# Farofeiro231/LiDAR_SLAM

Hardware: AMD Instinct MI355X
Metric: scans/sec (RANSAC+UKF, 720-pt scans) at 1/2/4/8 MI355X + HBM GB/s vs peak (higher is better)
Workload: dtype f64; 1 GPU; C3: 4096 synthetic 720-pt scans per GPU, chunked 7x100+20; RANSAC (100 trials, 20 mm, mt19937 hypotheses) + landmark association + UKF predict/update (n=3, L=20); scans_per_gpu=4096, trials=100, landmarks=20, hyp=mt19937, parallelism=dp1 (scan shards, no collective)

## Files before the change

lidar_slam_amd/csrc/lidarslam.hip:

```cpp
#include <hip/hip_runtime.h>
#include <math.h>
#include "lslam_host_math.h"
#include <stdio.h>
#include <stdlib.h>
#include <string.h>
#include <algorithm>
#include <atomic>
#include <mutex>
#include <new>
#include <string>
#include <vector>

#include "../../include/lidarslam.h"
#include "lslam_express.h"
#include "lslam_rng.h"
#include "lslam_rng_pipe.h"
#include "lslam_ransac.h"
#include "lslam_ukf.h"
#include "lslam_wave.h"

using namespace lslam;

static_assert(sizeof(lslam_chunk_model) == 112, "chunk model ABI");

__device__ __attribute__((noinline)) double2 polar_xy(double th, double d) {
    const double ang = -th * (LS_PI / 180.0) + LS_PI / 2.0;
    return make_double2(d * cos(ang), d * sin(ang));
}

struct PtSrc {
    const double2 *xy;
    const double *th, *dd;
    __device__ __forceinline__ double2 operator[](int64_t i) const { return xy ? xy[i] : polar_xy(th[i], dd[i]); }
    __device__ __forceinline__ PtSrc operator+(int64_t o) const {
        PtSrc r = *this;
        if (xy) r.xy += o;
        else { r.th += o; r.dd += o; }
        return r;
    }
};
__device__ __forceinline__ PtSrc batch_points(const lslam_scan_batch &B) {
    return PtSrc{(const double2 *)B.xy, B.theta_deg, B.dist_mm};
}
__device__ __forceinline__ void stage_points(const lslam_scan_batch &B, int p0, int N, double2 *P, int lane) {
    if (B.xy) {
        const double2 *src = (const double2 *)B.xy + p0;
        for (int p = lane; p < N; p += 64) P[p] = src[p];
    } else {
        for (int p = lane; p < N; p += 64) P[p] = polar_xy(B.theta_deg[p0 + p], B.dist_mm[p0 + p]);
    }
}
static_assert(sizeof(lslam_landmark) == 56, "landmark ABI");

__device__ __forceinline__ int owning_scan(const lslam_scan_batch &B, int c) {
    const int g = (int)(((int64_t)c * B.n_scans) / (B.n_chunks > 0 ? B.n_chunks : 1));
    if (g < B.n_scans && B.scan_chunk_off[g] <= c && c < B.scan_chunk_off[g + 1]) return uni(g);
    int lo = 0, hi = B.n_scans;
    while (hi - lo > 1) {
        const int mid = (lo + hi) >> 1;
        if (B.scan_chunk_off[mid] <= c) lo = mid;
        else hi = mid;
    }
    return uni(lo);
}

enum { MODE_RANSAC = 1, MODE_ASSOC = 2, MODE_UKF = 4, MODE_HYP_ONLY = 8, MODE_POST = 16 };

typedef float cut_t;
struct ChunkCut {
    double tq;
    double margin;
    cut_t c_lo, c_hi;
    int finite;
    int scan;
};

struct KArgs {
    lslam_scan_batch b;
    double ecut;
    double ecut_q;
    double thr;
    double tol_a, tol_b, tol_dist;
    double tol_dist_sq;
    uint64_t philox_seed;
    int T;
    int hyp_source;
    int life;
    int off_pts, off_key, off_ring, off_draws, off_cnt, off_tied, off_tsum;
    int off_vstack, off_nstack, off_snap, off_lmk, off_vis, off_mask, off_corg, off_zobs;
    int corg_cap;
    int off_recs;
    int off_ukf;
    int off_j1;
    int pts_cap;
    int lmk_cap;
    int hist_cap;
    UkfConst ukf;
    void *jbuf;
    int j8;
    int res_g;
    int32_t *draws_scr;
    uint32_t *state_scr;
    int off_blk, off_nxt, off_vtmp, off_stage;
    int rng_pipe_bytes;
    int off_stbl;
    const uint32_t *rt_all;
    const uint32_t *seed_state;
    int ep_d0, ep_nd;
    int ep_count;
    size_t slot_jbytes;
    int fixup;
    const uint8_t *spec_dirty_in;
    uint8_t *spec_dirty_out;
    int write_yproj;
    int lmk_reg;
    int32_t *cnt_scr;
    double *models;
    int cnt_blocks;
    const ChunkCut *cuts;
    unsigned long long *dbg;
    unsigned long long *wcen;
    unsigned int *wcen_n;
    unsigned int wcen_cap;
    unsigned int call_seq;
};

enum { WC_RNG_PARSER = 1, WC_RNG_HELPER, WC_RESOLVE, WC_CHUNK, WC_FIXUP, WC_POST, WC_UKF };
#if defined(LSLAM_STAMPS) || defined(LSLAM_CENSUS)
struct WaveCensus {
    const KArgs &a;
    uint32_t kid;
    uint64_t t0;
    __device__ WaveCensus(const KArgs &a_, uint32_t kid_) : a(a_), kid(kid_), t0(__builtin_amdgcn_s_memrealtime()) {}
    __device__ ~WaveCensus() {
        if (!a.wcen || (threadIdx.x & 63) != 0) return;
        const uint64_t t1 = __builtin_amdgcn_s_memrealtime();
// ... 132 lines not shown
        const int p = pb + lane;
        const double2 q = P[p < N ? p : 0];
        const bool h = p < N && resid2(q, mw) < ecut;
        const uint64_t bm = ballot(h);
        if (p < N) mk[p] = h ? 1 : 0;
        if (h) P[nin + (int)mbcnt(bm)] = q;
        nin += popc64(bm);
    }
    __syncthreads();
    o.n_inl = nin;
    o.last_inl = nin - 1;
    if (nin == 0) {
        o.flags |= LSLAM_NO_INLIERS;
        return o;
    }
    if (nin == 1) {
        o.flags |= LSLAM_EST_FAIL;
        return o;
    }
    const Model f = (nin == 2) ? model2(P[0], P[1]) : refit_line(P, nin, lane);
    o.m = f;
    o.flags |= LSLAM_VALID;
    if (f.ux == 0.0) o.flags |= LSLAM_VERTICAL;
    return o;
}

__device__ __forceinline__ double tie_bound(double S, int N, double E2) {
    return ((double)N * E2 + (double)(N + 32) * S) * 0x1p-42;
}

__device__ __forceinline__ double tie_bound_r(double S, int N, double E2, double R) {
    return ((double)N * (E2 + R * (sqrt(E2) + 1.0)) + (double)(N + 32) * S) * 0x1p-42;
}
__device__ __forceinline__ double tie_bound_q(double S, int N, double tq) {
    return ((double)N * tq + (double)(N + 32) * S) * 0x1p-42;
}

typedef unsigned u32x16 __attribute__((ext_vector_type(16)));
typedef unsigned u32x4 __attribute__((ext_vector_type(4)));

template <int OFF = 0>
__device__ __forceinline__ u32x16 sload_4pts(const double2 *p) {
    u32x16 v;
    asm volatile("s_load_dwordx16 %0, %1, %2" : "=s"(v) : "s"(p), "i"(OFF) : "memory");
    return v;
}
__device__ __forceinline__ u32x4 sload_pt(const double2 *p) {
    u32x4 v;
    asm volatile("s_load_dwordx4 %0, %1, 0x0" : "=s"(v) : "s"(p) : "memory");
    return v;
}
__device__ __forceinline__ void swait(u32x16 &v) { asm volatile("s_waitcnt lgkmcnt(0)" : "+s"(v)::"memory"); }
__device__ __forceinline__ void swait(u32x4 &v) { asm volatile("s_waitcnt lgkmcnt(0)" : "+s"(v)::"memory"); }
__device__ __forceinline__ double sd(unsigned lo, unsigned hi) {
    return __longlong_as_double((long long)(((unsigned long long)hi << 32) | lo));
}

__device__ __forceinline__ cut_t count_cut(double c) { return __uint_as_float((uint32_t)(__double_as_longlong(c) >> 32)); }
__device__ __forceinline__ bool sure_in(double r, cut_t c) { return __builtin_fabsf(count_cut(r)) < c; }
__device__ __forceinline__ bool maybe_in(double r, cut_t c) { return __builtin_fabsf(count_cut(r)) <= c; }
__device__ __forceinline__ void count_one(double x, double y, double ux, double uy, double k, cut_t c_lo,
                                          cut_t c_hi, int &lo, int &hi, double &S) {
    double t, r;
    asm("v_fma_f64 %0, %1, %2, %3" : "=v"(t) : "s"(y), "v"(ux), "v"(k));
    asm("v_fma_f64 %0, %1, %2, -%3" : "=v"(r) : "s"(x), "v"(uy), "v"(t));
    S = __builtin_fma(r, r, S);
    lo += sure_in(r, c_lo) ? 1 : 0;
    hi += maybe_in(r, c_hi) ? 1 : 0;
    asm volatile("" : "+v"(lo), "+v"(hi));
}

__device__ __forceinline__ void count_four(const u32x16 &A, double ux, double uy, double k, cut_t c_lo, cut_t c_hi,
                                           int &lo, int &hi, double &S) {
    asm volatile(
        "v_fma_f64 v[40:41], %[y0], %[ux], %[k]\n\t"
        "v_fma_f64 v[42:43], %[y1], %[ux], %[k]\n\t"
        "v_fma_f64 v[44:45], %[y2], %[ux], %[k]\n\t"
        "v_fma_f64 v[46:47], %[y3], %[ux], %[k]\n\t"
        "v_fma_f64 v[40:41], %[x0], %[uy], -v[40:41]\n\t"
        "v_fma_f64 v[42:43], %[x1], %[uy], -v[42:43]\n\t"
        "v_fma_f64 v[44:45], %[x2], %[uy], -v[44:45]\n\t"
        "v_fma_f64 v[46:47], %[x3], %[uy], -v[46:47]\n\t"
        "v_cmp_lt_f32_e64 s[80:81], |v41|, %[cl]\n\t"
        "v_cmp_le_f32_e64 s[82:83], |v41|, %[ch]\n\t"
        "v_cmp_lt_f32_e64 s[84:85], |v43|, %[cl]\n\t"
        "v_cmp_le_f32_e64 s[86:87], |v43|, %[ch]\n\t"
        "v_fma_f64 %[S], v[40:41], v[40:41], %[S]\n\t"
        "v_addc_co_u32_e64 %[lo], s[80:81], %[lo], 0, s[80:81]\n\t"
        "v_addc_co_u32_e64 %[hi], s[82:83], %[hi], 0, s[82:83]\n\t"
        "v_fma_f64 %[S], v[42:43], v[42:43], %[S]\n\t"
        "v_cmp_lt_f32_e64 s[80:81], |v45|, %[cl]\n\t"
        "v_cmp_le_f32_e64 s[82:83], |v45|, %[ch]\n\t"
        "v_addc_co_u32_e64 %[lo], s[84:85], %[lo], 0, s[84:85]\n\t"
        "v_addc_co_u32_e64 %[hi], s[86:87], %[hi], 0, s[86:87]\n\t"
        "v_fma_f64 %[S], v[44:45], v[44:45], %[S]\n\t"
        "v_cmp_lt_f32_e64 s[84:85], |v47|, %[cl]\n\t"
        "v_cmp_le_f32_e64 s[86:87], |v47|, %[ch]\n\t"
        "v_addc_co_u32_e64 %[lo], s[80:81], %[lo], 0, s[80:81]\n\t"
        "v_addc_co_u32_e64 %[hi], s[82:83], %[hi], 0, s[82:83]\n\t"
        "v_fma_f64 %[S], v[46:47], v[46:47], %[S]\n\t"
        "v_addc_co_u32_e64 %[lo], s[84:85], %[lo], 0, s[84:85]\n\t"
        "v_addc_co_u32_e64 %[hi], s[86:87], %[hi], 0, s[86:87]"
        : [lo] "+v"(lo), [hi] "+v"(hi), [S] "+v"(S)
        : [x0] "s"(sd(A[0], A[1])), [y0] "s"(sd(A[2], A[3])), [x1] "s"(sd(A[4], A[5])), [y1] "s"(sd(A[6], A[7])),
          [x2] "s"(sd(A[8], A[9])), [y2] "s"(sd(A[10], A[11])), [x3] "s"(sd(A[12], A[13])),
          [y3] "s"(sd(A[14], A[15])), [ux] "v"(ux), [uy] "v"(uy), [k] "v"(k), [cl] "v"(c_lo), [ch] "v"(c_hi)
        : "v40", "v41", "v42", "v43", "v44", "v45", "v46", "v47", "s80", "s81", "s82", "s83", "s84", "s85", "s86",
          "s87");
}

__device__ __forceinline__ void count_points_sgpr(const double2 *gP, int N, double ux, double uy, double k,
                                                  cut_t r_lo, cut_t r_hi, int &lo, int &hi, double &S) {
    const double2 *q = gP;
    if (N >= 8) {
        const double2 *const qlast = gP + ((N >> 3) - 1) * 8;
        u32x16 A = sload_4pts(q), B;
        swait(A);
        while (q != qlast) {
            B = sload_4pts<64>(q);
            count_four(A, ux, uy, k, r_lo, r_hi, lo, hi, S);
            swait(B);
            A = sload_4pts<128>(q);
            count_four(B, ux, uy, k, r_lo, r_hi, lo, hi, S);
            q += 8;
            swait(A);
        }
        B = sload_4pts<64>(q);
        count_four(A, ux, uy, k, r_lo, r_hi, lo, hi, S);
        swait(B);
        count_four(B, ux, uy, k, r_lo, r_hi, lo, hi, S);
        q += 8;
    }
    if (N & 4) {
        u32x16 A = sload_4pts(q);
        swait(A);
        count_four(A, ux, uy, k, r_lo, r_hi, lo, hi, S);
        q += 4;
    }
    for (int r = N & 3; r > 0; r--, q++) {
        u32x4 v = sload_pt(q);
        swait(v);
        count_one(sd(v[0], v[1]), sd(v[2], v[3]), ux, uy, k, r_lo, r_hi, lo, hi, S);
    }
}

__device__ __forceinline__ void count_points_lds(const double2 *P, int N, double ux, double uy, double k, cut_t r_lo,
                                                 cut_t r_hi, int &lo, int &hi, double &S) {
    int p = 0;
    for (; p + 2 <= N; p += 2) {
        const double2 q0 = P[p], q1 = P[p + 1];
        count_one(q0.x, q0.y, ux, uy, k, r_lo, r_hi, lo, hi, S);
        count_one(q1.x, q1.y, ux, uy, k, r_lo, r_hi, lo, hi, S);
    }
    if (p < N) count_one(P[p].x, P[p].y, ux, uy, k, r_lo, r_hi, lo, hi, S);
}

#ifdef LSLAM_STAMPS
#define CH_STAMP(k)                                                            \
    do {                                                                       \
        const uint64_t _t = lslam_stamp();                                     \
        if (chdbg && lane == 0) chdbg[(k)] += _t - _ch_prev;                   \
        _ch_prev = _t;                                                         \
    } while (0)
#define CH_STAMP_DECL uint64_t _ch_prev = lslam_stamp();
#define CH_STAMP_DECL_RESET _ch_prev = lslam_stamp();
#elif defined(LSLAM_CHUNK_EXIT)
#define CH_STAMP_DECL_RESET
#define CH_STAMP(k)                                           \
    do {                                                      \
        if ((k) == LSLAM_CHUNK_EXIT) asm volatile("s_endpgm"); \
    } while (0)
#define CH_STAMP_DECL
#else
#define CH_STAMP_DECL_RESET
#define CH_STAMP(k) do {} while (0)
#define CH_STAMP_DECL
#endif

__device__ __forceinline__ int hkey(double d) {
    const int h = (int)(__double_as_longlong(d) >> 32);
    return h ^ ((h >> 31) & 0x7fffffff);
}
__device__ __forceinline__ double key_up(int k) {
    const int h = k ^ ((k >> 31) & 0x7fffffff);
    return __longlong_as_double((long long)(((unsigned long long)(uint32_t)h << 32) | (h >= 0 ? 0xffffffffull : 0ull)));
}
__device__ __forceinline__ bool key_finite(int k) {
    const int h = k ^ ((k >> 31) & 0x7fffffff);
    return (h & 0x7ff00000) != 0x7ff00000;
}
struct BoxAcc {
    int xh = INT_MIN, xl = INT_MAX, yh = INT_MIN, yl = INT_MAX;
    __device__ __forceinline__ void add(double2 q) {
        const int kx = hkey(q.x), ky = hkey(q.y);
        xh = max(xh, kx);
        xl = min(xl, kx);
        yh = max(yh, ky);
        yl = min(yl, ky);
    }
};
__device__ __forceinline__ ChunkCut cut_finish(BoxAcc b, double ecut, double ecut_q);
template <typename PP>
__device__ __forceinline__ ChunkCut chunk_cut(PP P, int N, double ecut, double ecut_q, int lane) {
    BoxAcc b;
    for (int p = lane; p < N; p += 64) b.add(P[p]);
    return cut_finish(b, ecut, ecut_q);
}

template <int CTRL, int ROWS>
// ... 13 lines not shown
__device__ __forceinline__ float hi_units(double s, int d) {
    return __uint_as_float((uint32_t)(__double_as_longlong(s) >> 32) + (uint32_t)d);
}
__device__ __forceinline__ cut_t cut_lo_of(double e) {
    if (!(e > 0.0)) return -1.0f;
    if (e >= 0x1p-100 && e <= 0x1p100) return hi_units((double)__builtin_amdgcn_sqrtf((float)e), -2);
    return count_cut(sq_floor_lt(e));
}
__device__ __forceinline__ cut_t cut_hi_of(double e) {
    if (e >= 0x1p-100 && e <= 0x1p100) return hi_units((double)__builtin_amdgcn_sqrtf((float)e), 2);
    return count_cut(sq_ceil_gt(e));
}

__device__ __forceinline__ ChunkCut cut_from_keys(int kxh, int kxl, int kyh, int kyl, double ecut, double ecut_q) {
    ChunkCut cc;
    cc.finite = key_finite(kxh) && key_finite(kxl) && key_finite(kyh) && key_finite(kyl);
    const double hx = key_up(kxh), lx = key_up(kxl), hy = key_up(kyh), ly = key_up(kyl);
    const double bx = hx + lx, by = hy + ly;
    const double E2 = (bx * bx + by * by) * (1.0 + 0x1p-20);
    const double Rb = (fmax(hx, lx) + fmax(hy, ly)) * (1.0 + 0x1p-40);
    cc.finite = cc.finite && E2 < __builtin_inf();
    cc.scan = 0;
    cc.tq = 0.0;
    cc.margin = 0.0;
    cc.c_lo = count_cut(-1.0);
    cc.c_hi = count_cut(0.0);
    if (cc.finite && ecut < __builtin_inf()) {
        cc.margin = (E2 + ecut + Rb * ecut_q) * 0x1p-42;
        cc.c_lo = cut_lo_of(ecut - cc.margin);
        cc.c_hi = cut_hi_of(ecut + cc.margin);
        const double sE = (double)__builtin_amdgcn_sqrtf((float)E2) * (1.0 + 0x1p-20);
        cc.tq = E2 + Rb * (sE + 1.0);
    }
    return cc;
}
__device__ __forceinline__ ChunkCut cut_finish(BoxAcc b, double ecut, double ecut_q) {
    return cut_from_keys(wave_max_dpp(b.xh), wave_max_dpp(~b.xl), wave_max_dpp(b.yh), wave_max_dpp(~b.yl), ecut,
                         ecut_q);
}

__device__ ChunkOut chunk_consensus(const KArgs &a, double2 *P, const double2 *gP, int N, const int32_t *draws,
                                    int32_t *cnt, int32_t *tied, double *tsum, uint8_t *mk, double *vtmp,
                                    double *vstack, int *nstack, int32_t *cnt_out, int lane, const ChunkCut *pcut,
                                    unsigned long long *chdbg = nullptr) {
    CH_STAMP_DECL
    const int T = a.T;
    const double ecut = a.ecut;
    const ChunkCut cc = pcut ? *pcut : chunk_cut(P, N, ecut, a.ecut_q, lane);
    if (N > 128 || !cc.finite || !(ecut < __builtin_inf()))
        return chunk_ransac(a, P, N, draws, cnt, tied, tsum, mk, vstack, nstack, cnt_out, lane);

    ChunkOut o;
    o.flags = 0;
    o.best = -1;
    o.stop = -1;
    o.n_inl = 0;
    o.last_inl = -1;
    o.n_draws = T + 1;
    const double margin = cc.margin;
    const cut_t c_lo = cc.c_lo, c_hi = cc.c_hi;
    int M = 0;
    CH_STAMP(1);
    for (int tb = 0; tb < T; tb += 64) {
        const int t = tb + lane;
        const int tt = t < T ? t : 0;
        const Model m = model2(P[draws[2 * tt]], P[draws[2 * tt + 1]]);
        const double un = m.ux * m.ux + m.uy * m.uy;
        const bool exact_all = !(fabs(un - 1.0) <= 0x1p-46);
        const double k = __builtin_fma(m.ox, m.uy, -(m.oy * m.ux));
        int lo = 0, hi = 0;
        double S = 0.0;
        if (gP) count_points_sgpr(gP, N, m.ux, m.uy, k, c_lo, c_hi, lo, hi, S);
        else count_points_lds(P, N, m.ux, m.uy, k, c_lo, c_hi, lo, hi, S);
        int c = lo;
        if (exact_all || lo != hi) {
            c = 0;
            for (int q = 0; q < N; q++) {
                const double r = __builtin_fma(P[q].x, m.uy, -__builtin_fma(P[q].y, m.ux, k));
                const double v = r * r;
                bool in = v < ecut;
                if (exact_all || fabs(v - ecut) <= margin) in = resid2(P[q], m) < ecut;
                c += (int)in;
            }
        }
        if (t < T) {
            cnt[t] = c;
            tsum[t] = exact_all ? -1.0 : S;
            if (cnt_out) cnt_out[t] = c;
        }
        M = max(M, wave_max_dpp(t < T ? c : 0));
    }
    M = uni(M);
    CH_STAMP(2);
    __syncthreads();
    int ntied = 0;
    for (int tb = 0; tb < T; tb += 64) {
        const int t = tb + lane;
        const bool h = t < T && cnt[t] == M;
        const uint64_t bm = ballot(h);
        if (h) tied[ntied + (int)mbcnt(bm)] = t;
        ntied += popc64(bm);
    }
    __syncthreads();
    int best = -1;
    if (T > 0) {
        const bool need_sums = ntied > 1 || M == N || !(ecut > 0.0);
        if (!need_sums) {
            best = tied[0];
        } else {
            double U = __builtin_inf();
            for (int k = lane; k < ntied; k += 64) {
                const double S = tsum[tied[k]];
                if (S >= 0.0) U = fmin(U, S + tie_bound_q(S, N, cc.tq));
            }
            U = wave_min_d(U);
            int ncand = 0, cand1 = -1;
            for (int kb = 0; kb < ntied; kb += 64) {
                const int k = kb + lane;
                bool cand = false;
                if (k < ntied) {
                    const double S = tsum[tied[k]];
                    cand = S < 0.0 || S - tie_bound_q(S, N, cc.tq) <= U;
                }
                const uint64_t cm = ballot(cand);
                if (cm && cand1 < 0) cand1 = kb + ffs64(cm);
                ncand += popc64(cm);
            }
            const bool lone = ncand == 1 && M < N && ecut > 0.0;
            if (lone) best = uni(tied[cand1]);
            int bcnt = 0;
            double bsum = __builtin_inf();
            for (int kb = 0; !lone && kb < ntied && o.stop < 0; kb += 64) {
                const int k = kb + lane;
                bool cand = false;
                if (k < ntied) {
                    const double S = tsum[tied[k]];
                    cand = S < 0.0 || S - tie_bound_q(S, N, cc.tq) <= U;
                }
                uint64_t cm = ballot(cand);
                while (cm) {
                    const int bit = ffs64(cm);
                    cm &= cm - 1ull;
                    const int t = uni(tied[kb + bit]);
                    const Model m = model2(P[draws[2 * t]], P[draws[2 * t + 1]]);
                    const double s = pw_sum_regs(P, N, m, lane);
                    if (M > bcnt || (M == bcnt && s < bsum)) {
                        best = t;
                        bcnt = M;
                        bsum = s;
                        if (bsum <= 0.0) {
                            o.stop = t;
                            break;
                        }
                    }
                }
            }
        }
    }
    CH_STAMP(3);
    const ChunkOut of = chunk_finish_fit(a, P, N, draws, mk, uni(best), o, lane);
    CH_STAMP(4);
    return of;
}

__device__ bool finish_chunk(const KArgs &a, const ChunkOut &o, const double2 *P, uint8_t *mk, int p0, int N,
                             lslam_chunk_model &rec, int lane) {
    const lslam_scan_batch &B = a.b;
    const bool valid = (o.flags & LSLAM_VALID) != 0;
    if (!valid)
        for (int p = lane; p < N; p += 64) mk[p] = 0;
    __syncthreads();
    if (B.inlier_mask)
        for (int p = lane; p < N; p += 64) B.inlier_mask[p0 + p] = mk[p];
    rec.n_inliers = valid ? o.n_inl : 0;
    rec.best_trial = o.best;
    rec.n_draws = o.n_draws;
    rec.flags = o.flags;
    if (valid) {
// ... 888 lines not shown
    constexpr int wpg = 4;
    const int nwaves = (k.b.n_scans + per - 1) / per;
    const dim3 grid((unsigned)((nwaves + wpg - 1) / wpg)), block(64 * wpg);
    const int var = (trace ? UKF_VAR_TRACE : 0) | (k.b.ukf_sigmas ? UKF_VAR_SIGMAS : 0);
    switch (fuse ? 0 : var) {
        case 0: hipLaunchKernelGGL(ukf_group_kernel<0>, grid, block, 0, stream, k, Pg, fuse ? 1 : 0, nullptr); break;
        case 1: hipLaunchKernelGGL(ukf_group_kernel<1>, grid, block, 0, stream, k, Pg, 0, trace); break;
        case 2: hipLaunchKernelGGL(ukf_group_kernel<2>, grid, block, 0, stream, k, Pg, 0, nullptr); break;
        default: hipLaunchKernelGGL(ukf_group_kernel<3>, grid, block, 0, stream, k, Pg, 0, trace); break;
    }
}

__global__ __launch_bounds__(64) void seed_kernel(const uint32_t *__restrict__ seeds, int S, uint32_t *__restrict__ out) {
    __builtin_amdgcn_s_setprio(2);
    const int s = (int)blockIdx.x * 64 + (int)threadIdx.x;
    if (s >= S) return;
    uint32_t x = seeds ? seeds[s] : 0u;
    uint32_t *row = out + (size_t)s * MT_N;
#pragma unroll 8
    for (int i = 0; i < MT_N; i++) {
        row[i] = x;
        x = 1812433253u * (x ^ (x >> 30)) + (uint32_t)(i + 1);
    }
}

__global__ __launch_bounds__(64) void cut_lane_kernel(const KArgs a, ChunkCut *__restrict__ out) {
    __builtin_amdgcn_s_setprio(2);
    const lslam_scan_batch &B = a.b;
    const int c = (int)blockIdx.x * 64 + (int)threadIdx.x;
    if (c >= B.n_chunks) return;
    const int p0 = B.chunk_pt_off[c];
    const int N = B.chunk_pt_off[c + 1] - p0;
    BoxAcc b;
    if (B.xy) {
        const double2 *src = (const double2 *)B.xy + p0;
#pragma unroll 4
        for (int p = 0; p < N; p++) b.add(src[p]);
    } else {
        for (int p = 0; p < N; p++) b.add(polar_xy(B.theta_deg[p0 + p], B.dist_mm[p0 + p]));
    }
    ChunkCut cc = cut_from_keys(b.xh, ~b.xl, b.yh, ~b.yl, a.ecut, a.ecut_q);
    int g = (int)(((int64_t)c * B.n_scans) / (B.n_chunks > 0 ? B.n_chunks : 1));
    if (!(g < B.n_scans && B.scan_chunk_off[g] <= c && c < B.scan_chunk_off[g + 1])) {
        int lo = 0, hi = B.n_scans;
        while (hi - lo > 1) {
            const int mid = (lo + hi) >> 1;
            if (B.scan_chunk_off[mid] <= c) lo = mid;
            else hi = mid;
        }
        g = lo;
    }
    cc.scan = g;
    out[c] = cc;
}

constexpr int RNG_PPW = 4;
template <typename JT>
__global__ __launch_bounds__(64 * RNG_PPW) void rng_kernel(const KArgs a) {
    extern __shared__ __attribute__((aligned(16))) unsigned char smem[];
    const int lane = (int)threadIdx.x & 63;
    const int wave = uni((int)threadIdx.x >> 6);
    const lslam_scan_batch &B = a.b;
    const uint32_t D = a.ep_nd > 0 ? (uint32_t)a.ep_nd : (uint32_t)a.T + 1u;
    WAVE_CENSUS(a, WC_RNG_PARSER);
    RngPipe rp;
    {
        unsigned char *base = smem + (size_t)wave * a.rng_pipe_bytes;
        rp.blk = (uint32_t *)(base + a.off_blk);
        rp.have = 0;
        rp.tbl = nullptr;
        rp.tblK = 0;
    }
    int *kslot = (int *)(smem + a.off_stbl);
    uint32_t *stbl = (uint32_t *)(smem + a.off_stbl + 16);
// ... 454 lines not shown
            }
        };
        uint32_t rawA[RW], rawB[RW];
        if (2u <= K) load_group(2u, rawA);
        for (uint32_t ib = 2; ib <= K; ib += 128u * RW) {
            const uint32_t ib2 = ib + 64u * RW;
            if (ib2 <= K) load_group(ib2, rawB);
            walk_group(ib, rawA);
            if (ib2 > K) break;
            if (ib2 + 64u * RW <= K) load_group(ib2 + 64u * RW, rawA);
            walk_group(ib2, rawB);
        }
        if (lane == 0) {
            const uint32_t j1 = (uint32_t)Jd[K - 1u] & 1u;
            int32_t *draws = a.draws_scr + (size_t)c * 2 * Dall + 2 * (size_t)a.ep_d0;
            draws[2 * d] = (int32_t)((j1 == 0u) ? c1 : c0);
            draws[2 * d + 1] = (int32_t)((j1 == 0u) ? c0 : c1);
        }
    }
}

template <int HYP>
__device__ __forceinline__ void chunk_body(const KArgs &a, const int c, unsigned char *smem) {
    const int lane = (int)threadIdx.x;
    const lslam_scan_batch &B = a.b;
    double2 *P = (double2 *)(smem + a.off_pts);
    int32_t *draws = (int32_t *)(smem + a.off_draws);
    int32_t *cnt = (int32_t *)(smem + a.off_cnt);
    int32_t *tied = (int32_t *)(smem + a.off_tied);
    double *tsum = (double *)(smem + a.off_tsum);
    uint8_t *mk = (uint8_t *)(smem + a.off_mask);
    double *vstack = (double *)(smem + a.off_vstack);
    int *nstack = (int *)(smem + a.off_nstack);
    double *vtmp = (double *)(smem + a.off_vtmp);

    const int s = a.cuts ? uni(a.cuts[c].scan) : owning_scan(B, c);
    const int p0 = B.chunk_pt_off[c];
    const int N = B.chunk_pt_off[c + 1] - p0;
    const int T = a.T;
#ifdef LSLAM_STAMPS
    unsigned long long *chdbg = a.dbg ? a.dbg + (size_t)c * 16 : nullptr;
#else
    unsigned long long *chdbg = nullptr;
#endif
    CH_STAMP_DECL
    lslam_chunk_model rec;
    memset(&rec, 0, sizeof(rec));
    rec.best_trial = -1;
    rec.match_index = -1;
    rec.landmark_id = (B.id_base ? B.id_base[s] : 0) + (c - B.scan_chunk_off[s]);
    rec.n_points = N;
    if (N < 3) {
        rec.flags = LSLAM_N_TOO_SMALL;
        if (lane == 0 && B.models) B.models[c] = rec;
        for (int p = lane; p < N; p += 64) {
            if (B.inlier_mask) B.inlier_mask[p0 + p] = 0;
            if (B.y_proj && a.write_yproj) B.y_proj[p0 + p] = 0.0;
        }
        if (B.trial_cnt_out)
            for (int t = lane; t < a.T; t += 64) B.trial_cnt_out[(size_t)c * a.T + t] = 0;
        return;
    }
    const int D = T + 1;
    const int32_t *dr = draws;
    if (HYP == LSLAM_HYP_PHILOX) {
        philox_draws((uint32_t)N, (uint32_t)D, (uint32_t)c, a.philox_seed, draws, lane);
        if (B.draws_out)
            for (int i = lane; i < 2 * D; i += 64) B.draws_out[(size_t)c * 2 * D + i] = draws[i];
    } else {
        const int32_t *h = (HYP == LSLAM_HYP_EXPLICIT ? B.hyp : a.draws_scr) + (size_t)c * 2 * D;
        dr = h;
        if (N <= 128 && B.xy) {
            double2 pv[2];
            const double2 *src = (const double2 *)B.xy + p0;
#pragma unroll
            for (int k = 0; k < 2; k++) pv[k] = (lane + 64 * k < N) ? src[lane + 64 * k] : make_double2(0.0, 0.0);
#pragma unroll
            for (int k = 0; k < 2; k++)
                if (lane + 64 * k < N) P[lane + 64 * k] = pv[k];
        } else {
            stage_points(B, p0, N, P, lane);
        }
        if (HYP == LSLAM_HYP_EXPLICIT && B.draws_out)
            for (int i = lane; i < 2 * D; i += 64) B.draws_out[(size_t)c * 2 * D + i] = h[i];
    }
    CH_STAMP(0);
    if (HYP == LSLAM_HYP_PHILOX) stage_points(B, p0, N, P, lane);
    __syncthreads();
    CH_STAMP(6);
    const double2 *gP = B.xy ? (const double2 *)B.xy + p0 : nullptr;
    const ChunkOut o = chunk_consensus(a, P, gP, N, dr, cnt, tied, tsum, mk, vtmp, vstack, nstack,
                                       B.trial_cnt_out ? B.trial_cnt_out + (size_t)c * T : nullptr, lane,
                                       a.cuts ? a.cuts + c : nullptr, chdbg);
    CH_STAMP_DECL_RESET
    const bool have_model = finish_chunk(a, o, P, mk, p0, N, rec, lane);
    if (B.y_proj && a.write_yproj) chunk_yproj(B.y_proj + p0, P, mk, N, have_model, rec.proj_a, rec.proj_b, lane);
    if (lane == 0 && B.models) B.models[c] = rec;
    CH_STAMP(5);
}

template <int HYP>
__global__ __launch_bounds__(64, 4) void chunk_kernel(const KArgs a) {
    extern __shared__ __attribute__((aligned(16))) unsigned char smem[];
    WAVE_CENSUS(a, WC_CHUNK);
    for (int c = blockIdx.x; c < a.b.n_chunks; c += gridDim.x) {
        chunk_body<HYP>(a, c, smem);
        __syncthreads();
    }
}

constexpr int CNT_TPB = 256;
constexpr int CNT_HYP_BLOCK = 1024;

typedef const __attribute__((address_space(4))) double cdouble_t;

struct ChunkBox {
    double E2;
    bool finite;
};

template <typename Src>
__device__ __forceinline__ void box_partial(const Src src, int N, int tid, int nthr, double2 *P, double &xmn,
                                            double &xmx, double &ymn, double &ymx, bool &fin) {
    xmn = __builtin_inf(); xmx = -__builtin_inf(); ymn = __builtin_inf(); ymx = -__builtin_inf();
// ... 397 lines not shown
```

lidar_slam_amd/csrc/lslam_launch.h:

```cpp
#pragma once
#include <type_traits>

static inline int align16(int x) { return (x + 15) & ~15; }

template <typename F>
static void with_hyp_source(int hyp_source, F &&f) {
    switch (hyp_source) {
        case LSLAM_HYP_PHILOX: f(std::integral_constant<int, LSLAM_HYP_PHILOX>{}); break;
        case LSLAM_HYP_EXPLICIT: f(std::integral_constant<int, LSLAM_HYP_EXPLICIT>{}); break;
        default: f(std::integral_constant<int, LSLAM_HYP_MT19937>{}); break;
    }
}

static int validate_batch(const lslam_scan_batch *b, bool need_points) {
    if (!b) return set_err(LSLAM_ERR_ARG, "batch is NULL");
    if (b->n_scans < 0 || b->n_chunks < 0 || b->n_points < 0) return set_err(LSLAM_ERR_ARG, "negative sizes");
    if (b->n_scans == 0) return LSLAM_OK;
    if (!b->scan_chunk_off || !b->chunk_pt_off) return set_err(LSLAM_ERR_ARG, "missing CSR offsets");
    if (need_points && !b->xy && (!b->theta_deg || !b->dist_mm) && b->n_points > 0)
        return set_err(LSLAM_ERR_ARG, "missing points (xy, or theta_deg + dist_mm)");
    if (b->max_chunk_points < 0 || b->max_scan_chunks < 0) return set_err(LSLAM_ERR_ARG, "bad maxima");
    return LSLAM_OK;
}

// ... 26 lines not shown
#if defined(LSLAM_STAMPS) || defined(LSLAM_CENSUS)
    k.wcen = g_wcen;
    k.wcen_n = g_wcen_n;
    k.wcen_cap = g_wcen_cap;
    k.call_seq = g_call_seq;
#endif
    k.b = *b;
    if (p) {
        if (p->min_samples != 2) return set_err(LSLAM_ERR_UNSUPPORTED, "only min_samples == 2 (ransac_functions.py:11)");
        if (p->residual_threshold < 0) return set_err(LSLAM_ERR_ARG, "`residual_threshold` must be greater than zero");
        if (p->max_trials < 0) return set_err(LSLAM_ERR_ARG, "`max_trials` must be greater than zero");
        if (p->max_trials > 65533) return set_err(LSLAM_ERR_UNSUPPORTED, "max_trials > 65533");
        if (p->hyp_source < 0 || p->hyp_source > 2) return set_err(LSLAM_ERR_ARG, "bad hyp_source");
        if (p->hyp_source == LSLAM_HYP_EXPLICIT && !b->hyp) return set_err(LSLAM_ERR_ARG, "explicit hyp without hyp");
        k.thr = p->residual_threshold;
        k.ecut = lslam_inlier_cutoff(p->residual_threshold);
        k.ecut_q = std::sqrt(k.ecut) * 1.01 + 1.0;
        k.tol_a = p->tol_a;
        k.tol_b = p->tol_b;
        k.tol_dist = p->tol_dist;
        k.tol_dist_sq = sqrt_le_bound(p->tol_dist);
        k.philox_seed = p->philox_seed;
        k.T = p->max_trials;
        k.hyp_source = p->hyp_source;
        k.life = p->life;
    }
    if ((mode & MODE_ASSOC) && b->landmarks && !b->lmk_count) return set_err(LSLAM_ERR_ARG, "landmarks without lmk_count");
    const int N = b->max_chunk_points > 0 ? b->max_chunk_points : 1;
    const int T = k.T;
    int off = 0;
    if (mode & (MODE_RANSAC | MODE_HYP_ONLY)) {
        k.off_pts = off; off += align16(16 * N);
        k.off_key = off; off += align16(4 * 624);
        const int nxt_bytes = 4 * mt_nslot(N) * N;
        const int uni_bytes = max(nxt_bytes, 8 * (T > 0 ? T : 1));
        k.off_ring = off;
        k.off_tsum = off;
        off += align16(uni_bytes);
        k.off_j1 = off;
        off += align16(4 * mt_nslot(N));
        k.off_draws = off; off += align16(8 * (T + 1));
        k.off_cnt = off; off += align16(4 * (T > 0 ? T : 1));
        k.off_tied = off; off += align16(4 * (T > 0 ? T : 1));
        k.off_mask = off; off += align16(N);
        k.off_vstack = off; off += (N > 128) ? align16(8 * 64 * 24) : 0;
        k.off_nstack = off; off += (N > 128) ? align16(4 * 72) : 0;
        k.off_recs = -1;
    } else {
        k.off_mask = off; off += align16(N);
        const int msc = b->max_scan_chunks > 0 ? b->max_scan_chunks : 1;
        if (msc <= 256) {
            k.off_recs = off;
            off += align16((int)sizeof(lslam_chunk_model) * msc) + align16(4 * (msc + 1));
        } else {
            k.off_recs = -1;
        }
    }
    if (u && u->n_landmarks > 0) {
        k.off_ukf = 0;
        off = max(off, align16(8 * UkfLds::doubles(u->n_landmarks)));
    }
    k.hist_cap = b->max_scan_chunks > 0 ? b->max_scan_chunks : 1;
    k.off_snap = off; off += (mode & MODE_RANSAC) ? align16(4 * MT_N) : 0;
    k.corg_cap = k.hist_cap;
    k.off_corg = off; off += align16(16 * k.corg_cap);
    k.off_zobs = off; off += (u && (u->flags & LSLAM_UKF_MAP)) ? align16(16 * k.corg_cap) : 0;
    k.lmk_cap = (mode & MODE_ASSOC) ? b->lmk_capacity : 0;
    if ((mode & MODE_ASSOC) && k.lmk_cap <= 0) return set_err(LSLAM_ERR_ARG, "lmk_capacity must be > 0");
    k.lmk_reg = (mode == MODE_ASSOC && k.lmk_cap > 0 && k.lmk_cap <= 64 && k.off_recs >= 0 &&
                 !(u && (u->flags & LSLAM_UKF_MAP)) && b->landmarks) ? 1 : 0;
    k.off_lmk = off; off += k.lmk_reg ? 0 : align16((int)sizeof(lslam_landmark) * (k.lmk_cap > 0 ? k.lmk_cap : 1));
    k.off_vis = off; off += k.lmk_reg ? 0 : align16(8 * ((k.lmk_cap + 63) / 64 + 1));
    k.pts_cap = N;
// ... 41 lines not shown
        const int mx = 160 * 1024;
        (void)hipFuncSetAttribute((const void *)scan_kernel<0, MODE>, hipFuncAttributeMaxDynamicSharedMemorySize, mx);
        (void)hipFuncSetAttribute((const void *)scan_kernel<1, MODE>, hipFuncAttributeMaxDynamicSharedMemorySize, mx);
        (void)hipFuncSetAttribute((const void *)scan_kernel<2, MODE>, hipFuncAttributeMaxDynamicSharedMemorySize, mx);
        set_max_lds(scan_kernel_w4<LSLAM_HYP_EXPLICIT, MODE>);
    });
    int st = timer_begin(c, timer);
    if (st) return st;
    if (MODE == MODE_UKF && !(k.ukf.flags & LSLAM_UKF_MAP)) {
        launch_ukf_group(k, k.ukf.L, c->stream, false);
        HIPCHK(hipGetLastError());
    } else if (MODE == MODE_ASSOC || MODE == MODE_UKF) {
        hipLaunchKernelGGL((scan_kernel_w4<LSLAM_HYP_EXPLICIT, MODE>), dim3((unsigned)k.b.n_scans), dim3(64), lds,
                           c->stream, k);
        HIPCHK(hipGetLastError());
    } else {
        HIPCHK(launch_mode<MODE>(k, lds, c->stream));
    }
    st = timer_end(c, timer);
    if (st) return st;
    return LSLAM_OK;
}


static int layout_chunk(KArgs &k, const lslam_scan_batch *b, int &lds) {
    const int N = b->max_chunk_points > 0 ? b->max_chunk_points : 1;
    const int T = k.T;
    int off = 0;
    k.off_pts = off; off += align16(16 * N);
    k.off_draws = off; off += (k.hyp_source == LSLAM_HYP_PHILOX) ? align16(8 * (T + 1)) : 0;
    k.off_cnt = off; off += align16(4 * (T > 0 ? T : 1));
    k.off_tied = off; off += align16(4 * (T > 0 ? T : 1));
    k.off_tsum = off; off += align16(8 * (T > 0 ? T : 1));
    k.off_mask = off; off += align16(N);
    k.off_vstack = off; off += (N > 128) ? align16(8 * 64 * 24) : 0;
    k.off_nstack = off; off += (N > 128) ? align16(4 * 72) : 0;
    k.off_vtmp = off;
    lds = off;
    if (lds > 160 * 1024) return set_err(LSLAM_ERR_CAPACITY, "chunk/trial sizes exceed the 160 KiB LDS");
    return LSLAM_OK;
}

static int layout_rng(KArgs &k, const lslam_scan_batch *b, int &lds) {
    const int N = b->max_chunk_points > 3 ? b->max_chunk_points : 3;
    if (N > 65536) return set_err(LSLAM_ERR_UNSUPPORTED, "chunks of more than 65536 points");
    int off = 0;
    k.off_blk = off; off += align16(4 * (2 * 624 + 64));
    k.rng_pipe_bytes = off;
    lds = off * RNG_PPW;
    k.off_stbl = lds;
    lds += 16 + 2 * 4 * RT_DWORDS;
    return LSLAM_OK;
}

static inline unsigned launch_cap(int64_t n) { return (unsigned)(n < (1 << 30) ? (n > 0 ? n : 1) : (1 << 30)); }

template <typename F>
static void set_max_lds(F *fn) {
    hipFuncAttributes at;
    size_t stat = 0;
    if (hipFuncGetAttributes(&at, (const void *)fn) == hipSuccess) stat = at.sharedSizeBytes;
    (void)hipFuncSetAttribute((const void *)fn, hipFuncAttributeMaxDynamicSharedMemorySize, (int)(160 * 1024 - stat));
    (void)hipGetLastError();
}

static int prepare_steps(lslam_ctx *c, KArgs &k, int slot) {
// ... 656 lines not shown
```

lidar_slam_amd/csrc/lslam_rng.h:

```cpp
#pragma once
#include "lslam_wave.h"

namespace lslam {

__device__ __forceinline__ void wave_lds_sync() {
    __builtin_amdgcn_wave_barrier();
    asm volatile("" ::: "memory");
}

constexpr int MT_N = 624;
constexpr int MT_M = 397;
constexpr uint32_t MT_UP = 0x80000000u;
constexpr uint32_t MT_LO = 0x7fffffffu;
constexpr uint32_t MT_MA = 0x9908b0dfu;

__device__ __forceinline__ uint32_t mt_temper(uint32_t y) {
    y ^= (y >> 11);
    y ^= (y << 7) & 0x9d2c5680u;
    y ^= (y << 15) & 0xefc60000u;
    y ^= (y >> 18);
    return y;
}

__device__ __forceinline__ uint32_t mt_mix(uint32_t cur, uint32_t nxt, uint32_t far) {
// ... 75 lines not shown
};

constexpr uint32_t MT_NONE = 0xffffffffu;

#ifdef LSLAM_STAMPS
__device__ __forceinline__ uint64_t lslam_stamp() {
    uint64_t t;
    __builtin_amdgcn_sched_barrier(0);
    asm volatile("s_memtime %0\n\ts_waitcnt lgkmcnt(0)" : "=s"(t)::"memory");
    __builtin_amdgcn_sched_barrier(0);
    return t;
}
#define LSLAM_STAMP_DECL uint64_t _st_prev = lslam_stamp();
#define LSLAM_STAMP(k)                         \
    do {                                       \
        const uint64_t _t = lslam_stamp();     \
        mt.acc[k] += _t - _st_prev;            \
        _st_prev = _t;                         \
    } while (0)
#else
#define LSLAM_STAMP_DECL
#define LSLAM_STAMP(k) \
    do {               \
    } while (0)
#endif

__host__ __device__ inline int mt_resolve_batch(int N) { return N <= 512 ? 4 : 1; }
__host__ __device__ inline int mt_nslot(int N) {
    const int K = N > 2 ? N - 1 : 2;
    int need = mt_resolve_batch(N) + (64 + K - 1) / K;
    int s = 1;
    while (s < need) s <<= 1;
    return s;
}

__device__ __forceinline__ uint32_t nxt_tag(uint32_t d) { return (0xfffeu - d) << 16; }

__device__ __forceinline__ void mt_resolve(const MTWave &mt, uint32_t N, uint32_t smask, uint32_t d0, uint32_t nb,
                                           int32_t *draws, int lane) {
    const uint32_t k = (uint32_t)lane >> 1;
    const uint32_t q = (uint32_t)lane & 1u;
    uint32_t p = q;
    const uint32_t d = d0 + k;
    const uint32_t slot = d & smask;
    const uint32_t tag = nxt_tag(d);
    if (k < nb) {
        const uint32_t *nx = mt.nxt + slot * N;
        for (;;) {
            const uint32_t t = nx[p];
            if ((t & 0xffff0000u) != tag) break;
            p = t & 0xffffu;
        }
    }
    const uint32_t other = (uint32_t)__shfl_xor((int)p, 1);
    if (k < nb && q == 0) {
        const uint32_t j1 = mt.j1s[slot];
        const uint32_t a0 = (j1 == 0u) ? other : p;
        const uint32_t a1 = (j1 == 0u) ? p : other;
        draws[2 * d] = (int32_t)a0;
        draws[2 * d + 1] = (int32_t)a1;
    }
    wave_lds_sync();
}

template <bool FAST>
__device__ void mt_draws_impl(MTWave &mt, uint32_t N, uint32_t D, int32_t *draws, bool store, int lane) {
// ... 147 lines not shown
```

Measured before the change: 6.261 million scans/s.

## Replace per-point residual sum accumulation with closed-form moment-based tie bracket

The inner RANSAC counting loop no longer accumulates the squared residual sum per point. Instead, per-chunk second moments are precomputed in the cut pass, and the sum of squared residuals for each hypothesis line is computed in closed form, together with a rigorous per-trial error bound stored as a float in LDS. This removes an FMA per point per trial from the hot counting loop. In exchange it adds moment accumulation in the prepass, a new LDS buffer and bound logic for tie-breaking. It also risks a fallback to the exact path more often when the bounds are loose, and a wave reduction when no precomputed cuts exist.

```diff
diff --git a/lidar_slam_amd/csrc/lidarslam.hip b/lidar_slam_amd/csrc/lidarslam.hip
--- a/lidar_slam_amd/csrc/lidarslam.hip
+++ b/lidar_slam_amd/csrc/lidarslam.hip
@@ -16,6 +16,7 @@
 #include "lslam_rng.h"
 #include "lslam_rng_pipe.h"
 #include "lslam_ransac.h"
+#include "lslam_tie_moments.h"
 #include "lslam_ukf.h"
 #include "lslam_wave.h"
 
@@ -73,7 +74,10 @@
     cut_t c_lo, c_hi;
     int finite;
     int scan;
+    TieMoments mom;
+    double tm_ok;
 };
+static_assert(sizeof(ChunkCut) == 96 && sizeof(ChunkCut) % 16 == 0, "ChunkCut: six 16-byte rows");
 
 struct KArgs {
     lslam_scan_batch b;
@@ -102,6 +106,7 @@
     int32_t *draws_scr;
     uint32_t *state_scr;
     int off_blk, off_nxt, off_vtmp, off_stage;
+    int off_tbnd;
     int rng_pipe_bytes;
     int off_stbl;
     const uint32_t *rt_all;
@@ -300,9 +305,6 @@
 __device__ __forceinline__ double tie_bound_r(double S, int N, double E2, double R) {
     return ((double)N * (E2 + R * (sqrt(E2) + 1.0)) + (double)(N + 32) * S) * 0x1p-42;
 }
-__device__ __forceinline__ double tie_bound_q(double S, int N, double tq) {
-    return ((double)N * tq + (double)(N + 32) * S) * 0x1p-42;
-}
 
 typedef unsigned u32x16 __attribute__((ext_vector_type(16)));
 typedef unsigned u32x4 __attribute__((ext_vector_type(4)));
@@ -328,18 +330,17 @@
 __device__ __forceinline__ bool sure_in(double r, cut_t c) { return __builtin_fabsf(count_cut(r)) < c; }
 __device__ __forceinline__ bool maybe_in(double r, cut_t c) { return __builtin_fabsf(count_cut(r)) <= c; }
 __device__ __forceinline__ void count_one(double x, double y, double ux, double uy, double k, cut_t c_lo,
-                                          cut_t c_hi, int &lo, int &hi, double &S) {
+                                          cut_t c_hi, int &lo, int &hi) {
     double t, r;
     asm("v_fma_f64 %0, %1, %2, %3" : "=v"(t) : "s"(y), "v"(ux), "v"(k));
     asm("v_fma_f64 %0, %1, %2, -%3" : "=v"(r) : "s"(x), "v"(uy), "v"(t));
-    S = __builtin_fma(r, r, S);
     lo += sure_in(r, c_lo) ? 1 : 0;
     hi += maybe_in(r, c_hi) ? 1 : 0;
     asm volatile("" : "+v"(lo), "+v"(hi));
 }
 
 __device__ __forceinline__ void count_four(const u32x16 &A, double ux, double uy, double k, cut_t c_lo, cut_t c_hi,
-                                           int &lo, int &hi, double &S) {
+                                           int &lo, int &hi) {
     asm volatile(
         "v_fma_f64 v[40:41], %[y0], %[ux], %[k]\n\t"
         "v_fma_f64 v[42:43], %[y1], %[ux], %[k]\n\t"
@@ -353,32 +354,28 @@
         "v_cmp_le_f32_e64 s[82:83], |v41|, %[ch]\n\t"
         "v_cmp_lt_f32_e64 s[84:85], |v43|, %[cl]\n\t"
         "v_cmp_le_f32_e64 s[86:87], |v43|, %[ch]\n\t"
-        "v_fma_f64 %[S], v[40:41], v[40:41], %[S]\n\t"
+        "v_cmp_lt_f32_e64 s[88:89], |v45|, %[cl]\n\t"
+        "v_cmp_le_f32_e64 s[90:91], |v45|, %[ch]\n\t"
         "v_addc_co_u32_e64 %[lo], s[80:81], %[lo], 0, s[80:81]\n\t"
         "v_addc_co_u32_e64 %[hi], s[82:83], %[hi], 0, s[82:83]\n\t"
-        "v_fma_f64 %[S], v[42:43], v[42:43], %[S]\n\t"
-        "v_cmp_lt_f32_e64 s[80:81], |v45|, %[cl]\n\t"
-        "v_cmp_le_f32_e64 s[82:83], |v45|, %[ch]\n\t"
+        "v_cmp_lt_f32_e64 s[80:81], |v47|, %[cl]\n\t"
+        "v_cmp_le_f32_e64 s[82:83], |v47|, %[ch]\n\t"
         "v_addc_co_u32_e64 %[lo], s[84:85], %[lo], 0, s[84:85]\n\t"
         "v_addc_co_u32_e64 %[hi], s[86:87], %[hi], 0, s[86:87]\n\t"
-        "v_fma_f64 %[S], v[44:45], v[44:45], %[S]\n\t"
-        "v_cmp_lt_f32_e64 s[84:85], |v47|, %[cl]\n\t"
-        "v_cmp_le_f32_e64 s[86:87], |v47|, %[ch]\n\t"
+        "v_addc_co_u32_e64 %[lo], s[88:89], %[lo], 0, s[88:89]\n\t"
+        "v_addc_co_u32_e64 %[hi], s[90:91], %[hi], 0, s[90:91]\n\t"
         "v_addc_co_u32_e64 %[lo], s[80:81], %[lo], 0, s[80:81]\n\t"
-        "v_addc_co_u32_e64 %[hi], s[82:83], %[hi], 0, s[82:83]\n\t"
-        "v_fma_f64 %[S], v[46:47], v[46:47], %[S]\n\t"
-        "v_addc_co_u32_e64 %[lo], s[84:85], %[lo], 0, s[84:85]\n\t"
-        "v_addc_co_u32_e64 %[hi], s[86:87], %[hi], 0, s[86:87]"
-        : [lo] "+v"(lo), [hi] "+v"(hi), [S] "+v"(S)
+        "v_addc_co_u32_e64 %[hi], s[82:83], %[hi], 0, s[82:83]"
+        : [lo] "+v"(lo), [hi] "+v"(hi)
         : [x0] "s"(sd(A[0], A[1])), [y0] "s"(sd(A[2], A[3])), [x1] "s"(sd(A[4], A[5])), [y1] "s"(sd(A[6], A[7])),
           [x2] "s"(sd(A[8], A[9])), [y2] "s"(sd(A[10], A[11])), [x3] "s"(sd(A[12], A[13])),
           [y3] "s"(sd(A[14], A[15])), [ux] "v"(ux), [uy] "v"(uy), [k] "v"(k), [cl] "v"(c_lo), [ch] "v"(c_hi)
         : "v40", "v41", "v42", "v43", "v44", "v45", "v46", "v47", "s80", "s81", "s82", "s83", "s84", "s85", "s86",
-          "s87");
+          "s87", "s88", "s89", "s90", "s91");
 }
 
 __device__ __forceinline__ void count_points_sgpr(const double2 *gP, int N, double ux, double uy, double k,
-                                                  cut_t r_lo, cut_t r_hi, int &lo, int &hi, double &S) {
+                                                  cut_t r_lo, cut_t r_hi, int &lo, int &hi) {
     const double2 *q = gP;
     if (N >= 8) {
         const double2 *const qlast = gP + ((N >> 3) - 1) * 8;
@@ -386,41 +383,41 @@
         swait(A);
         while (q != qlast) {
             B = sload_4pts<64>(q);
-            count_four(A, ux, uy, k, r_lo, r_hi, lo, hi, S);
+            count_four(A, ux, uy, k, r_lo, r_hi, lo, hi);
             swait(B);
             A = sload_4pts<128>(q);
-            count_four(B, ux, uy, k, r_lo, r_hi, lo, hi, S);
+            count_four(B, ux, uy, k, r_lo, r_hi, lo, hi);
             q += 8;
             swait(A);
         }
         B = sload_4pts<64>(q);
-        count_four(A, ux, uy, k, r_lo, r_hi, lo, hi, S);
+        count_four(A, ux, uy, k, r_lo, r_hi, lo, hi);
         swait(B);
-        count_four(B, ux, uy, k, r_lo, r_hi, lo, hi, S);
+        count_four(B, ux, uy, k, r_lo, r_hi, lo, hi);
         q += 8;
     }
     if (N & 4) {
         u32x16 A = sload_4pts(q);
         swait(A);
-        count_four(A, ux, uy, k, r_lo, r_hi, lo, hi, S);
+        count_four(A, ux, uy, k, r_lo, r_hi, lo, hi);
         q += 4;
     }
     for (int r = N & 3; r > 0; r--, q++) {
         u32x4 v = sload_pt(q);
         swait(v);
-        count_one(sd(v[0], v[1]), sd(v[2], v[3]), ux, uy, k, r_lo, r_hi, lo, hi, S);
+        count_one(sd(v[0], v[1]), sd(v[2], v[3]), ux, uy, k, r_lo, r_hi, lo, hi);
     }
 }
 
 __device__ __forceinline__ void count_points_lds(const double2 *P, int N, double ux, double uy, double k, cut_t r_lo,
-                                                 cut_t r_hi, int &lo, int &hi, double &S) {
+                                                 cut_t r_hi, int &lo, int &hi) {
     int p = 0;
     for (; p + 2 <= N; p += 2) {
         const double2 q0 = P[p], q1 = P[p + 1];
-        count_one(q0.x, q0.y, ux, uy, k, r_lo, r_hi, lo, hi, S);
-        count_one(q1.x, q1.y, ux, uy, k, r_lo, r_hi, lo, hi, S);
-    }
-    if (p < N) count_one(P[p].x, P[p].y, ux, uy, k, r_lo, r_hi, lo, hi, S);
+        count_one(q0.x, q0.y, ux, uy, k, r_lo, r_hi, lo, hi);
+        count_one(q1.x, q1.y, ux, uy, k, r_lo, r_hi, lo, hi);
+    }
+    if (p < N) count_one(P[p].x, P[p].y, ux, uy, k, r_lo, r_hi, lo, hi);
 }
 
 #ifdef LSLAM_STAMPS
@@ -432,6 +429,10 @@
     } while (0)
 #define CH_STAMP_DECL uint64_t _ch_prev = lslam_stamp();
 #define CH_STAMP_DECL_RESET _ch_prev = lslam_stamp();
+#define CH_COUNT(k, v)                                  \
+    do {                                                \
+        if (chdbg && lane == 0) chdbg[(k)] += (v);      \
+    } while (0)
 #elif defined(LSLAM_CHUNK_EXIT)
 #define CH_STAMP_DECL_RESET
 #define CH_STAMP(k)                                           \
@@ -443,6 +444,9 @@
 #define CH_STAMP_DECL_RESET
 #define CH_STAMP(k) do {} while (0)
 #define CH_STAMP_DECL
+#endif
+#ifndef CH_COUNT
+#define CH_COUNT(k, v) do {} while (0)
 #endif
 
 __device__ __forceinline__ int hkey(double d) {
@@ -522,6 +526,8 @@
         const double sE = (double)__builtin_amdgcn_sqrtf((float)E2) * (1.0 + 0x1p-20);
         cc.tq = E2 + Rb * (sE + 1.0);
     }
+    cc.mom = tie_mom_init(0.0, 0.0);
+    cc.tm_ok = (cc.finite && ecut < __builtin_inf() && tie_moments_usable(Rb, cc.tq)) ? 1.0 : 0.0;
     return cc;
 }
 __device__ __forceinline__ ChunkCut cut_finish(BoxAcc b, double ecut, double ecut_q) {
@@ -529,8 +535,23 @@
                          ecut_q);
 }
 
+__device__ __forceinline__ TieMoments wave_moments(const double2 *P, int N, int lane) {
+    TieMoments m = tie_mom_init(unid(P[0].x), unid(P[0].y));
+    for (int p = lane; p < N; p += 64) tie_mom_add(m, P[p].x, P[p].y);
+#pragma unroll
+    for (int o = 32; o > 0; o >>= 1)
+        tie_mom_merge(m, __shfl_xor(m.sx, o), __shfl_xor(m.sy, o), __shfl_xor(m.sxx, o), __shfl_xor(m.sxy, o),
+                      __shfl_xor(m.syy, o));
+    m.sx = unid(m.sx);
+    m.sy = unid(m.sy);
+    m.sxx = unid(m.sxx);
+    m.sxy = unid(m.sxy);
+    m.syy = unid(m.syy);
+    return m;
+}
+
 __device__ ChunkOut chunk_consensus(const KArgs &a, double2 *P, const double2 *gP, int N, const int32_t *draws,
-                                    int32_t *cnt, int32_t *tied, double *tsum, uint8_t *mk, double *vtmp,
+                                    int32_t *cnt, int32_t *tied, double *tsum, float *tbnd, uint8_t *mk,
                                     double *vstack, int *nstack, int32_t *cnt_out, int lane, const ChunkCut *pcut,
                                     unsigned long long *chdbg = nullptr) {
     CH_STAMP_DECL
@@ -539,6 +560,7 @@
     const ChunkCut cc = pcut ? *pcut : chunk_cut(P, N, ecut, a.ecut_q, lane);
     if (N > 128 || !cc.finite || !(ecut < __builtin_inf()))
         return chunk_ransac(a, P, N, draws, cnt, tied, tsum, mk, vstack, nstack, cnt_out, lane);
+    const bool tm_ok = cc.tm_ok != 0.0;
 
     ChunkOut o;
     o.flags = 0;
@@ -559,9 +581,11 @@
         const bool exact_all = !(fabs(un - 1.0) <= 0x1p-46);
         const double k = __builtin_fma(m.ox, m.uy, -(m.oy * m.ux));
         int lo = 0, hi = 0;
-        double S = 0.0;
-        if (gP) count_points_sgpr(gP, N, m.ux, m.uy, k, c_lo, c_hi, lo, hi, S);
-        else count_points_lds(P, N, m.ux, m.uy, k, c_lo, c_hi, lo, hi, S);
+        if (gP) count_points_sgpr(gP, N, m.ux, m.uy, k, c_lo, c_hi, lo, hi);
+        else count_points_lds(P, N, m.ux, m.uy, k, c_lo, c_hi, lo, hi);
+        const TieMoments mom = pcut ? pcut->mom : (tm_ok ? wave_moments(P, N, lane) : tie_mom_init(0.0, 0.0));
+        double Bh;
+        const double S = tie_bracket(mom, N, m.ox, m.oy, m.ux, m.uy, Bh);
         int c = lo;
         if (exact_all || lo != hi) {
             c = 0;
@@ -575,7 +599,8 @@
         }
         if (t < T) {
             cnt[t] = c;
-            tsum[t] = exact_all ? -1.0 : S;
+            tsum[t] = (exact_all || !tm_ok) ? -1.0 : S;
+            tbnd[t] = tie_bound_up(Bh);
             if (cnt_out) cnt_out[t] = c;
         }
         M = max(M, wave_max_dpp(t < T ? c : 0));
@@ -598,10 +623,12 @@
         if (!need_sums) {
             best = tied[0];
         } else {
+            CH_COUNT(8, ntied);
+            CH_COUNT(10, 1);
             double U = __builtin_inf();
             for (int k = lane; k < ntied; k += 64) {
                 const double S = tsum[tied[k]];
-                if (S >= 0.0) U = fmin(U, S + tie_bound_q(S, N, cc.tq));
+                if (S >= 0.0) U = fmin(U, S + (double)tbnd[tied[k]]);
             }
             U = wave_min_d(U);
             int ncand = 0, cand1 = -1;
@@ -610,7 +637,7 @@
                 bool cand = false;
                 if (k < ntied) {
                     const double S = tsum[tied[k]];
-                    cand = S < 0.0 || S - tie_bound_q(S, N, cc.tq) <= U;
+                    cand = S < 0.0 || S - (double)tbnd[tied[k]] <= U;
                 }
                 const uint64_t cm = ballot(cand);
                 if (cm && cand1 < 0) cand1 = kb + ffs64(cm);
@@ -625,7 +652,7 @@
                 bool cand = false;
                 if (k < ntied) {
                     const double S = tsum[tied[k]];
-                    cand = S < 0.0 || S - tie_bound_q(S, N, cc.tq) <= U;
+                    cand = S < 0.0 || S - (double)tbnd[tied[k]] <= U;
                 }
                 uint64_t cm = ballot(cand);
                 while (cm) {
@@ -634,6 +661,7 @@
                     const int t = uni(tied[kb + bit]);
                     const Model m = model2(P[draws[2 * t]], P[draws[2 * t + 1]]);
                     const double s = pw_sum_regs(P, N, m, lane);
+                    CH_COUNT(9, 1);
                     if (M > bcnt || (M == bcnt && s < bsum)) {
                         best = t;
                         bcnt = M;
@@ -1588,14 +1616,29 @@
     const int p0 = B.chunk_pt_off[c];
     const int N = B.chunk_pt_off[c + 1] - p0;
     BoxAcc b;
+    TieMoments mom = tie_mom_init(0.0, 0.0);
     if (B.xy) {
         const double2 *src = (const double2 *)B.xy + p0;
+        if (N > 0) mom = tie_mom_init(src[0].x, src[0].y);
 #pragma unroll 4
-        for (int p = 0; p < N; p++) b.add(src[p]);
+        for (int p = 0; p < N; p++) {
+            const double2 q = src[p];
+            b.add(q);
+            tie_mom_add(mom, q.x, q.y);
+        }
     } else {
-        for (int p = 0; p < N; p++) b.add(polar_xy(B.theta_deg[p0 + p], B.dist_mm[p0 + p]));
+        if (N > 0) {
+            const double2 q0 = polar_xy(B.theta_deg[p0], B.dist_mm[p0]);
+            mom = tie_mom_init(q0.x, q0.y);
+        }
+        for (int p = 0; p < N; p++) {
+            const double2 q = polar_xy(B.theta_deg[p0 + p], B.dist_mm[p0 + p]);
+            b.add(q);
+            tie_mom_add(mom, q.x, q.y);
+        }
     }
     ChunkCut cc = cut_from_keys(b.xh, ~b.xl, b.yh, ~b.yl, a.ecut, a.ecut_q);
+    cc.mom = mom;
     int g = (int)(((int64_t)c * B.n_scans) / (B.n_chunks > 0 ? B.n_chunks : 1));
     if (!(g < B.n_scans && B.scan_chunk_off[g] <= c && c < B.scan_chunk_off[g + 1])) {
         int lo = 0, hi = B.n_scans;
@@ -2116,7 +2159,7 @@
     uint8_t *mk = (uint8_t *)(smem + a.off_mask);
     double *vstack = (double *)(smem + a.off_vstack);
     int *nstack = (int *)(smem + a.off_nstack);
-    double *vtmp = (double *)(smem + a.off_vtmp);
+    float *tbnd = (float *)(smem + a.off_tbnd);
 
     const int s = a.cuts ? uni(a.cuts[c].scan) : owning_scan(B, c);
     const int p0 = B.chunk_pt_off[c];
@@ -2173,7 +2216,7 @@
     __syncthreads();
     CH_STAMP(6);
     const double2 *gP = B.xy ? (const double2 *)B.xy + p0 : nullptr;
-    const ChunkOut o = chunk_consensus(a, P, gP, N, dr, cnt, tied, tsum, mk, vtmp, vstack, nstack,
+    const ChunkOut o = chunk_consensus(a, P, gP, N, dr, cnt, tied, tsum, tbnd, mk, vstack, nstack,
                                        B.trial_cnt_out ? B.trial_cnt_out + (size_t)c * T : nullptr, lane,
                                        a.cuts ? a.cuts + c : nullptr, chdbg);
     CH_STAMP_DECL_RESET
diff --git a/lidar_slam_amd/csrc/lslam_launch.h b/lidar_slam_amd/csrc/lslam_launch.h
--- a/lidar_slam_amd/csrc/lslam_launch.h
+++ b/lidar_slam_amd/csrc/lslam_launch.h
@@ -82,13 +82,13 @@
     if (mode & (MODE_RANSAC | MODE_HYP_ONLY)) {
         k.off_pts = off; off += align16(16 * N);
         k.off_key = off; off += align16(4 * 624);
-        const int nxt_bytes = 4 * mt_nslot(N) * N;
+        const int nxt_bytes = 4 * mt_nxt_entries_max(N);
         const int uni_bytes = max(nxt_bytes, 8 * (T > 0 ? T : 1));
         k.off_ring = off;
         k.off_tsum = off;
         off += align16(uni_bytes);
         k.off_j1 = off;
-        off += align16(4 * mt_nslot(N));
+        off += align16(4 * mt_nslot_max(N));
         k.off_draws = off; off += align16(8 * (T + 1));
         k.off_cnt = off; off += align16(4 * (T > 0 ? T : 1));
         k.off_tied = off; off += align16(4 * (T > 0 ? T : 1));
@@ -196,6 +196,7 @@
     k.off_cnt = off; off += align16(4 * (T > 0 ? T : 1));
     k.off_tied = off; off += align16(4 * (T > 0 ? T : 1));
     k.off_tsum = off; off += align16(8 * (T > 0 ? T : 1));
+    k.off_tbnd = off; off += align16(4 * (T > 0 ? T : 1));
     k.off_mask = off; off += align16(N);
     k.off_vstack = off; off += (N > 128) ? align16(8 * 64 * 24) : 0;
     k.off_nstack = off; off += (N > 128) ? align16(4 * 72) : 0;
diff --git a/lidar_slam_amd/csrc/lslam_rng.h b/lidar_slam_amd/csrc/lslam_rng.h
--- a/lidar_slam_amd/csrc/lslam_rng.h
+++ b/lidar_slam_amd/csrc/lslam_rng.h
@@ -131,6 +131,15 @@
     int s = 1;
     while (s < need) s <<= 1;
     return s;
+}
+__host__ __device__ inline int mt_nslot_max(int N) { return mt_nslot(N < 3 ? N : 3); }
+__host__ __device__ inline int mt_nxt_entries_max(int N) {
+    int m = mt_nslot(N) * N;
+    for (int n = 3; n < N && n <= 512; n++) {
+        const int e = mt_nslot(n) * n;
+        m = e > m ? e : m;
+    }
+    return m;
 }
 
 __device__ __forceinline__ uint32_t nxt_tag(uint32_t d) { return (0xfffeu - d) << 16; }
diff --git a/lidar_slam_amd/csrc/lslam_tie_moments.h b/lidar_slam_amd/csrc/lslam_tie_moments.h
--- /dev/null
+++ b/lidar_slam_amd/csrc/lslam_tie_moments.h
@@ -0,0 +1,76 @@
+#pragma once
+#include <cmath>
+
+#if defined(__HIPCC__)
+#define LSLAM_TM_FN __host__ __device__ __forceinline__
+#else
+#define LSLAM_TM_FN static inline
+#endif
+
+struct TieMoments {
+    double cx, cy;
+    double sx, sy;
+    double sxx, sxy, syy;
+};
+
+LSLAM_TM_FN TieMoments tie_mom_init(double cx, double cy) {
+    TieMoments m;
+    m.cx = cx; m.cy = cy;
+    m.sx = m.sy = m.sxx = m.sxy = m.syy = 0.0;
+    return m;
+}
+
+LSLAM_TM_FN void tie_mom_add(TieMoments &m, double x, double y) {
+    const double ax = x - m.cx, ay = y - m.cy;
+    m.sx += ax;
+    m.sy += ay;
+    m.sxx = __builtin_fma(ax, ax, m.sxx);
+    m.sxy = __builtin_fma(ax, ay, m.sxy);
+    m.syy = __builtin_fma(ay, ay, m.syy);
+}
+
+LSLAM_TM_FN void tie_mom_merge(TieMoments &m, double sx, double sy, double sxx, double sxy, double syy) {
+    m.sx += sx;
+    m.sy += sy;
+    m.sxx += sxx;
+    m.sxy += sxy;
+    m.syy += syy;
+}
+
+LSLAM_TM_FN TieMoments tie_moments_seq(const double *xy, int N) {
+    TieMoments m = tie_mom_init(N > 0 ? xy[0] : 0.0, N > 0 ? xy[1] : 0.0);
+    for (int p = 0; p < N; p++) tie_mom_add(m, xy[2 * p], xy[2 * p + 1]);
+    return m;
+}
+
+LSLAM_TM_FN double tie_bracket(const TieMoments &m, int N, double ox, double oy, double ux, double uy, double &B,
+                               double scale = 1.0) {
+    const double n = (double)N;
+    const double bx = ox - m.cx, by = oy - m.cy;
+    const double kp = __builtin_fma(bx, uy, -(by * ux));
+    const double t1 = (uy * uy) * m.sxx;
+    const double t2 = (ux * uy) * m.sxy;
+    const double t3 = (ux * ux) * m.syy;
+    const double t4 = n * (kp * kp);
+    const double t5 = kp * __builtin_fma(uy, m.sx, -(ux * m.sy));
+    double s = ((t1 - 2.0 * t2) + t3) + (t4 - 2.0 * t5);
+    s = s > 0.0 ? s : 0.0;
+    const double V = (m.sxx + m.syy) + n * __builtin_fma(bx, bx, by * by);
+    double W = V - 2.0 * __builtin_fma(bx, m.sx, by * m.sy);
+    W = W > 0.0 ? W : 0.0;
+    B = scale * ((166.0 * W + n * s) + (2.01 * n + 26.0) * V) * 0x1p-53;
+    return s;
+}
+
+LSLAM_TM_FN float tie_bound_up(double B) {
+    float f = (float)B;
+    if ((double)f < B) {
+        unsigned bits;
+        __builtin_memcpy(&bits, &f, 4);
+        bits += 1u;
+        __builtin_memcpy(&f, &bits, 4);
+    }
+    return f < 0x1p-126f ? 0x1p-126f : f;
+}
+
+LSLAM_TM_FN bool tie_moments_usable(double R, double tq) { return R <= 0x1p40 && tq >= 0x1p-400; }
```

Result: no change. 6.258 million scans/s (-0.0%).
